# DeepLearnPhysics/dynamic-gcnn

Measured on AMD Instinct MI355X. Metric: point-clouds/sec fwd+bwd at (B,N,k,C)=(24,2048,20,3), 1/2/4/8 MI355X, higher is better.
Workload: dtype f32

## Files before the change

dynamic-gcnn_amd/csrc/bn.hip:

```cpp
#include "common.h"
#include <stdlib.h>

namespace {

constexpr int FIN_COLS = 4, FIN_LANES = 64;
__device__ __forceinline__ bool slot_sums(const double* __restrict__ acc, int F, int nslots, int& f, double& s, double& q,
                                          int colblock) {
  const int c = threadIdx.x / FIN_LANES, z = threadIdx.x % FIN_LANES;
  f = colblock * FIN_COLS + c;
  if (f >= F) return false;
  double a = 0.0, b = 0.0;
  int sl = z;
  for (; sl + 3 * FIN_LANES < nslots; sl += 4 * FIN_LANES) {
    double va[4], vb[4];
#pragma unroll
    for (int u = 0; u < 4; ++u) {
      va[u] = acc[((int64_t)(sl + u * FIN_LANES) * 2 + 0) * F + f];
      vb[u] = acc[((int64_t)(sl + u * FIN_LANES) * 2 + 1) * F + f];
    }
#pragma unroll
    for (int u = 0; u < 4; ++u) { a += va[u]; b += vb[u]; }
  }
  for (; sl < nslots; sl += FIN_LANES) {
    a += acc[((int64_t)sl * 2 + 0) * F + f];
// ... 68 lines not shown

struct Src {
  const float* Y;
  const float* V; int64_t ldv;
  const float* U; int64_t ldu;
  const int32_t* idx;
  unsigned npts;
};

#ifndef BN_NB
#define BN_NB 4
#endif
constexpr int CNT_POS = 256;
constexpr int NB = BN_NB;

template <int V, bool G>
struct Rows {
  const float* base;
  const int32_t* ip;
  int64_t ld;
  float u[V];
  __device__ __forceinline__ void init(const Src& s, int64_t r, int k, int F, int f) {
    if (G) {
      const unsigned cloud = (unsigned)r / s.npts;
      base = s.V + (int64_t)cloud * s.npts * s.ldv + f;
      ip = s.idx + r * k;
      ld = s.ldv;
      Vec<V>::ld(s.U + r * s.ldu + f, u);
    } else {
      base = s.Y + (r * k) * F + f;
      ip = nullptr;
      ld = F;
    }
  }
  __device__ __forceinline__ void load(int m, int k, float (&y)[NB][V]) const {
    if constexpr (G) {
      unsigned row[NB];
#pragma unroll
      for (int b = 0; b < NB; ++b) row[b] = __umul24((unsigned)ip[(m + b < k) ? (m + b) : (k - 1)], (unsigned)ld);
#pragma unroll
      for (int b = 0; b < NB; ++b) Vec<V>::ld(base + row[b], y[b]);
#pragma unroll
      for (int b = 0; b < NB; ++b)
#pragma unroll
        for (int v = 0; v < V; ++v) y[b][v] += u[v];
    } else {
#pragma unroll
      for (int b = 0; b < NB; ++b)
        if (m + b < k) Vec<V>::ld(base + (int64_t)(m + b) * ld, y[b]);
    }
  }
};

struct Items { int64_t base, count, first, step; };
template <bool G>
__device__ __forceinline__ Items items_of(int64_t R, int FV) {
  Items it;
  if (G) {
    const int64_t per = (R + 7) / 8;
    const int64_t rb = (int64_t)(blockIdx.x & 7) * per;
    int64_t rows = R - rb;
    rows = rows < 0 ? 0 : (rows > per ? per : rows);
    it.base = rb * FV;
    it.count = rows * FV;
    it.first = (int64_t)(blockIdx.x >> 3) * blockDim.x + threadIdx.x;
    it.step = (int64_t)(gridDim.x >> 3) * blockDim.x;
  } else {
    it.base = 0;
    it.count = R * FV;
    it.first = (int64_t)blockIdx.x * blockDim.x + threadIdx.x;
    it.step = (int64_t)gridDim.x * blockDim.x;
  }
  return it;
}

template <int V, bool G>
__global__ __launch_bounds__(256) void bn_act_kreduce_kernel(
    Src src, int64_t R, int k, int F, const float* __restrict__ mean,
    const float* __restrict__ rstd, const float* __restrict__ beta, int relu,
    float* __restrict__ max_out, int64_t ldmax, float* __restrict__ mean_out, int64_t ldmean,
    float* __restrict__ out2, int64_t ldout2, float* __restrict__ cnt_out, int fv_shift) {
  const int FV = F / V;
  const Items its = items_of<G>(R, FV);
  const float invk = 1.0f / (float)k;
  for (int64_t q = its.first; q < its.count; q += its.step) {
    int64_t r;
    int fq;
    split_item(its.base + q, FV, fv_shift, r, fq);
    const int f = fq * V;
    float mu[V], rs[V], be[V], mx[V], sm[V], cn[V], np[V];
    Vec<V>::ld(mean + f, mu); Vec<V>::ld(rstd + f, rs); Vec<V>::ld(beta + f, be);
#pragma unroll
    for (int v = 0; v < V; ++v) { mx[v] = -INFINITY; sm[v] = 0.f; cn[v] = 0.f; np[v] = 0.f; }
    Rows<V, G> rows;
    rows.init(src, r, k, F, f);
    for (int m = 0; m < k; m += NB) {
      float yv[NB][V];
      rows.load(m, k, yv);
#pragma unroll
      for (int b = 0; b < NB; ++b)
        if (m + b < k) {
#pragma unroll
          for (int v = 0; v < V; ++v) {
            float xh;
            const float z = bn_z(yv[b][v], mu[v], rs[v], be[v], relu, xh);
            const bool gt = z > mx[v];
            cn[v] = gt ? 1.f : ((z == mx[v]) ? cn[v] + 1.f : cn[v]);
            mx[v] = gt ? z : mx[v];
            sm[v] += z;
            if (G) np[v] += (z > 0.f) ? (float)CNT_POS : 0.f;
          }
        }
    }
    Vec<V>::st(max_out + r * ldmax + f, mx);
    if (out2) Vec<V>::st(out2 + r * ldout2 + f, mx);
    if (G) {
#pragma unroll
      for (int v = 0; v < V; ++v) cn[v] += np[v];
    }
    if (cnt_out) Vec<V>::st(cnt_out + r * F + f, cn);
    if (mean_out) {
#pragma unroll
      for (int v = 0; v < V; ++v) sm[v] *= invk;
      Vec<V>::st(mean_out + r * ldmean + f, sm);
    }
  }
}

template <int V>
struct KState { float mx[V]; float cnt[V]; };

template <int V, bool G>
__device__ __forceinline__ void k_pass_max(const Rows<V, G>& rows, int k, const float (&mu)[V],
                                           const float (&rs)[V], const float (&be)[V], int relu,
                                           KState<V>& st) {
#pragma unroll
  for (int v = 0; v < V; ++v) { st.mx[v] = -INFINITY; st.cnt[v] = 0.f; }
  for (int m = 0; m < k; m += NB) {
    float yv[NB][V];
    rows.load(m, k, yv);
#pragma unroll
    for (int b = 0; b < NB; ++b)
      if (m + b < k) {
#pragma unroll
        for (int v = 0; v < V; ++v) {
          float xh;
          const float z = bn_z(yv[b][v], mu[v], rs[v], be[v], relu, xh);
          if (z > st.mx[v]) { st.mx[v] = z; st.cnt[v] = 1.f; }
          else if (z == st.mx[v]) st.cnt[v] += 1.f;
        }
      }
  }
}

template <int V, bool G>
__global__ __launch_bounds__(256) void bn_bwd_reduce_kernel(
    Src src, int64_t R, int k, int F, const float* __restrict__ mean,
    const float* __restrict__ rstd, const float* __restrict__ beta, int relu,
    const float* __restrict__ dmax, int64_t lddmax, const float* __restrict__ dmean, int64_t lddmean,
    const float* __restrict__ mx_in, int64_t ldmx, const float* __restrict__ cnt_in, double* __restrict__ red,
    int fv_shift, int nslots) {
  extern __shared__ float lred[];
  for (int e = threadIdx.x; e < 2 * F; e += blockDim.x) lred[e] = 0.f;
  __syncthreads();
  const int FV = F / V;
  const Items its = items_of<G>(R, FV);
  const float invk = 1.0f / (float)k;
  int curf = -1;
  float s0[V], s1[V];
#pragma unroll
  for (int v = 0; v < V; ++v) { s0[v] = 0.f; s1[v] = 0.f; }
  for (int64_t q = its.first; q < its.count; q += its.step) {
    int64_t r;
    int fq;
    split_item(its.base + q, FV, fv_shift, r, fq);
    const int f = fq * V;
    if (f != curf) {
      if (curf >= 0) {
#pragma unroll
        for (int v = 0; v < V; ++v) { atomicAdd(&lred[curf + v], s0[v]); atomicAdd(&lred[F + curf + v], s1[v]); s0[v] = 0.f; s1[v] = 0.f; }
      }
      curf = f;
    }
    float mu[V], rs[V], be[V], dmx[V], dmn[V];
    Vec<V>::ld(mean + f, mu); Vec<V>::ld(rstd + f, rs); Vec<V>::ld(beta + f, be);
    Vec<V>::ld(dmax + r * lddmax + f, dmx);
    Rows<V, G> rows;
    rows.init(src, r, k, F, f);
    KState<V> st;
    if (dmean) {
      Vec<V>::ld(dmean + r * lddmean + f, dmn);
      if (mx_in) {
        Vec<V>::ld(mx_in + r * ldmx + f, st.mx);
        Vec<V>::ld(cnt_in + r * F + f, st.cnt);
        if (G) {
#pragma unroll
          for (int v = 0; v < V; ++v) st.cnt[v] -= (float)CNT_POS * floorf(st.cnt[v] * (1.0f / CNT_POS));
        }
      } else {
        k_pass_max<V, G>(rows, k, mu, rs, be, relu, st);
      }
    }
    for (int m = 0; m < k; m += NB) {
      float yv[NB][V];
      rows.load(m, k, yv);
#pragma unroll
      for (int b = 0; b < NB; ++b)
        if (m + b < k) {
#pragma unroll
          for (int v = 0; v < V; ++v) {
            float xh;
            const float z = bn_z(yv[b][v], mu[v], rs[v], be[v], relu, xh);
            float dz;
            if (dmean) dz = ((z == st.mx[v]) ? dmx[v] / st.cnt[v] : 0.f) + dmn[v] * invk;
            else dz = dmx[v];
            if (relu && !(z > 0.f)) dz = 0.f;
            s0[v] += dz;
            s1[v] += dz * xh;
          }
        }
    }
  }
  if (curf >= 0) {
#pragma unroll
    for (int v = 0; v < V; ++v) { atomicAdd(&lred[curf + v], s0[v]); atomicAdd(&lred[F + curf + v], s1[v]); }
  }
  __syncthreads();
  const int slot = blockIdx.x % nslots;
  for (int e = threadIdx.x; e < 2 * F; e += blockDim.x)
    atomicAdd(red + (int64_t)slot * 2 * F + e, (double)lred[e]);
}

template <int V, bool G>
__global__ __launch_bounds__(256) void bn_bwd_apply_kernel(
    Src src, int64_t R, int k, int F, const float* __restrict__ mean,
    const float* __restrict__ rstd, const float* __restrict__ beta, int relu,
    const float* __restrict__ dmax, int64_t lddmax, const float* __restrict__ dmean, int64_t lddmean,
    const float* __restrict__ mx_in, int64_t ldmx, const float* __restrict__ cnt_in,
    const double* __restrict__ red, float* dY, float* __restrict__ dYsum, int64_t lddysum, int fv_shift) {
  const bool round_dy = (relu & 2) != 0;
  relu &= 1;
  const int FV = F / V;
  const Items its = items_of<G>(R, FV);
  const float invk = 1.0f / (float)k;
  const double inv_cnt = 1.0 / ((double)R * (double)k);
  for (int64_t q = its.first; q < its.count; q += its.step) {
    int64_t r;
    int fq;
    split_item(its.base + q, FV, fv_shift, r, fq);
    const int f = fq * V;
    float mu[V], rs[V], be[V], dmx[V], dmn[V], c1[V], c2[V], acc[V];
    Vec<V>::ld(mean + f, mu); Vec<V>::ld(rstd + f, rs); Vec<V>::ld(beta + f, be);
    Vec<V>::ld(dmax + r * lddmax + f, dmx);
#pragma unroll
    for (int v = 0; v < V; ++v) {
      c1[v] = (float)(red[f + v] * inv_cnt);
      c2[v] = (float)(red[F + f + v] * inv_cnt);
      acc[v] = 0.f;
    }
    Rows<V, G> rows;
    rows.init(src, r, k, F, f);
    float* dy = dY + (r * k) * F + f;
    KState<V> st;
    if (dmean) {
      Vec<V>::ld(dmean + r * lddmean + f, dmn);
      if (mx_in) {
        Vec<V>::ld(mx_in + r * ldmx + f, st.mx);
        Vec<V>::ld(cnt_in + r * F + f, st.cnt);
        if (G) {
#pragma unroll
          for (int v = 0; v < V; ++v) st.cnt[v] -= (float)CNT_POS * floorf(st.cnt[v] * (1.0f / CNT_POS));
        }
      } else {
        k_pass_max<V, G>(rows, k, mu, rs, be, relu, st);
      }
    }
    for (int m = 0; m < k; m += NB) {
      float yv[NB][V];
      rows.load(m, k, yv);
#pragma unroll
      for (int b = 0; b < NB; ++b)
        if (m + b < k) {
          float o[V];
#pragma unroll
          for (int v = 0; v < V; ++v) {
            float xh;
            const float z = bn_z(yv[b][v], mu[v], rs[v], be[v], relu, xh);
            float dz;
            if (dmean) dz = ((z == st.mx[v]) ? dmx[v] / st.cnt[v] : 0.f) + dmn[v] * invk;
            else dz = dmx[v];
            if (relu && !(z > 0.f)) dz = 0.f;
            o[v] = rs[v] * (dz - c1[v] - xh * c2[v]);
            if (round_dy) o[v] = round_bf16_rne(o[v]);
            acc[v] += o[v];
          }
          Vec<V>::st(dy + (int64_t)(m + b) * F, o);
        }
    }
    if (dYsum) Vec<V>::st(dYsum + r * lddysum + f, acc);
  }
}


template <int CC>
__global__ __launch_bounds__(256) void edge_bwd_apply_wgrad_kernel(
    Src src, int64_t R, int k, int F, const float* __restrict__ mean, const float* __restrict__ rstd,
    const float* __restrict__ beta, const float* __restrict__ dmax, int64_t lddmax, const float* __restrict__ dmean,
    int64_t lddmean, const float* __restrict__ mx_in, int64_t ldmx, const float* __restrict__ cnt_in,
    const double* __restrict__ red, const float* __restrict__ x, int64_t ldx, int C, float* __restrict__ partial, int fv_shift) {
  constexpr int V = 4;
  extern __shared__ float sh[];
  const int FV = F / V;
  const Items its = items_of<true>(R, FV);
  const float invk = 1.0f / (float)k;
  const double inv_cnt = 1.0 / ((double)R * (double)k);
  float wc[CC][V], wd[CC][V];
#pragma unroll
  for (int c = 0; c < CC; ++c)
#pragma unroll
    for (int v = 0; v < V; ++v) { wc[c][v] = 0.f; wd[c][v] = 0.f; }
  const int fq_fixed = (int)((its.base + its.first) & (FV - 1));
  const int f = fq_fixed * V;
  float mu[V], rs[V], be[V], c1[V], c2[V];
  Vec<V>::ld(mean + f, mu); Vec<V>::ld(rstd + f, rs); Vec<V>::ld(beta + f, be);
#pragma unroll
  for (int v = 0; v < V; ++v) {
    c1[v] = (float)(red[f + v] * inv_cnt);
    c2[v] = (float)(red[F + f + v] * inv_cnt);
  }
  for (int64_t q = its.first; q < its.count; q += its.step) {
    const int64_t r = (its.base + q) >> fv_shift;
    float dmx[V], dmn[V];
    Vec<V>::ld(dmax + r * lddmax + f, dmx);
    Vec<V>::ld(dmean + r * lddmean + f, dmn);
    Rows<V, true> rows;
    rows.init(src, r, k, F, f);
    KState<V> st;
    Vec<V>::ld(mx_in + r * ldmx + f, st.mx);
    Vec<V>::ld(cnt_in + r * F + f, st.cnt);
#pragma unroll
    for (int v = 0; v < V; ++v) st.cnt[v] -= (float)CNT_POS * floorf(st.cnt[v] * (1.0f / CNT_POS));
    float xi[CC];
#pragma unroll
    for (int c = 0; c < CC; ++c) xi[c] = (c < C) ? x[r * ldx + c] : 0.f;
    const int64_t cloud0 = (int64_t)((unsigned)r / src.npts) * src.npts;
    float acc[V] = {0.f, 0.f, 0.f, 0.f};
    for (int m = 0; m < k; m += NB) {
      float yv[NB][V];
      rows.load(m, k, yv);
#pragma unroll
      for (int b = 0; b < NB; ++b)
        if (m + b < k) {
          const float* xj = x + (cloud0 + rows.ip[m + b]) * ldx;
          float dx[CC];
#pragma unroll
          for (int c = 0; c < CC; ++c) dx[c] = (c < C) ? xj[c] - xi[c] : 0.f;
#pragma unroll
          for (int v = 0; v < V; ++v) {
            float xh;
            const float z = bn_z(yv[b][v], mu[v], rs[v], be[v], 1, xh);
            float dz = ((z == st.mx[v]) ? dmx[v] / st.cnt[v] : 0.f) + dmn[v] * invk;
            if (!(z > 0.f)) dz = 0.f;
            const float o = rs[v] * (dz - c1[v] - xh * c2[v]);
            acc[v] += o;
#pragma unroll
            for (int c = 0; c < CC; ++c) wd[c][v] = fmaf(dx[c], o, wd[c][v]);
          }
        }
    }
#pragma unroll
    for (int c = 0; c < CC; ++c)
#pragma unroll
      for (int v = 0; v < V; ++v) wc[c][v] = fmaf(xi[c], acc[v], wc[c][v]);
  }
  const int lanes = 256 / FV;
  const int rl = threadIdx.x / FV;
#pragma unroll
  for (int c = 0; c < CC; ++c)
#pragma unroll
    for (int v = 0; v < V; ++v) {
      sh[(rl * 2 * CC + c) * F + f + v] = wc[c][v];
      sh[(rl * 2 * CC + CC + c) * F + f + v] = wd[c][v];
    }
  __syncthreads();
  float* out = partial + (int64_t)blockIdx.x * 2 * C * F;
  for (int e = threadIdx.x; e < 2 * CC * F; e += 256) {
    const int cr = e / F, ff = e % F;
    const int c = cr < CC ? cr : cr - CC;
    if (c >= C) continue;
    float s = 0.f;
    for (int l = 0; l < lanes; ++l) s += sh[(l * 2 * CC + cr) * F + ff];
    out[(int64_t)(cr < CC ? c : C + c) * F + ff] = s;
  }
}

struct K1Map {
  int f; int64_t r0, rstep; bool on;
};
__device__ __forceinline__ K1Map k1_map(int F, int FVB, int RP) {
  K1Map m;
  const int t = threadIdx.x;
  const int fq = blockIdx.y * 256 + (t % FVB);
  m.f = fq * 4;
  m.on = (t < RP * FVB) && (m.f < F);
  m.r0 = (int64_t)blockIdx.x * RP + t / FVB;
  m.rstep = (int64_t)gridDim.x * RP;
  return m;
}

constexpr int K1_PARK_FLOATS = 2048;
__device__ __forceinline__ void k1_block_sums(float* lpark, const K1Map& m, int F, int FVB, int RP, const float (&s0)[4],
                                              const float (&s1)[4], double* __restrict__ red, int nslots) {
  const int t = threadIdx.x;
  const int W = 4 * FVB;
  if (t < RP * FVB) {
    const int rp = t / FVB, cb = (t % FVB) * 4;
#pragma unroll
    for (int v = 0; v < 4; ++v) {
      lpark[(rp * 2 + 0) * W + cb + v] = m.on ? s0[v] : 0.f;
      lpark[(rp * 2 + 1) * W + cb + v] = m.on ? s1[v] : 0.f;
    }
  }
  __syncthreads();
  const int fbase = blockIdx.y * 1024;
  const int slot = blockIdx.x % nslots;
  for (int e = t; e < 2 * W; e += blockDim.x) {
    const int which = e / W, cb = e % W;
    if (fbase + cb < F) {
      float a = 0.f;
      for (int rp = 0; rp < RP; ++rp) a += lpark[(rp * 2 + which) * W + cb];
      atomicAdd(red + ((int64_t)slot * 2 + which) * F + fbase + cb, (double)a);
    }
  }
}

__global__ __launch_bounds__(256) void bn1_act_kernel(const float* __restrict__ T, int64_t R, int F, int FVB, int RP,
                                                      const float* __restrict__ mean, const float* __restrict__ rstd,
                                                      const float* __restrict__ beta, int relu,
                                                      float* __restrict__ out, int64_t ldo, float* __restrict__ out2,
                                                      int64_t ldo2, float* __restrict__ cnt_out,
                                                      const uint64_t* __restrict__ drop_seed, float drop_keep) {
  const K1Map m = k1_map(F, FVB, RP);
  if (!m.on) return;
  const uint64_t dseed = drop_seed ? *drop_seed : 0ull;
  const uint32_t dthr = dropout_threshold(drop_keep);
  const float dscale = drop_seed ? 1.0f / drop_keep : 1.0f;
  float mu[4], rs[4], be[4];
  Vec<4>::ld(mean + m.f, mu); Vec<4>::ld(rstd + m.f, rs); Vec<4>::ld(beta + m.f, be);
  const float one[4] = {1.f, 1.f, 1.f, 1.f};
  for (int64_t r = m.r0; r < R; r += 4 * m.rstep) {
    float y[4][4];
#pragma unroll
    for (int b = 0; b < 4; ++b) {
      const int64_t rr = r + b * m.rstep;
      if (rr < R) Vec<4>::ld(T + rr * F + m.f, y[b]);
    }
#pragma unroll
    for (int b = 0; b < 4; ++b) {
      const int64_t rr = r + b * m.rstep;
      if (rr < R) {
        float z[4];
#pragma unroll
        for (int v = 0; v < 4; ++v) { float xh; z[v] = bn_z(y[b][v], mu[v], rs[v], be[v], relu, xh); }
        if (drop_seed) {
#pragma unroll
          for (int v = 0; v < 4; ++v) z[v] = dropout_keeps(dseed, (uint64_t)(rr * F + m.f + v), dthr) ? z[v] * dscale : 0.f;
        }
        Vec<4>::st(out + rr * ldo + m.f, z);
        if (out2) Vec<4>::st(out2 + rr * ldo2 + m.f, z);
        if (cnt_out) Vec<4>::st(cnt_out + rr * F + m.f, one);
      }
    }
  }
}

template <bool APPLY>
__global__ __launch_bounds__(256) void bn1_bwd_kernel(const float* T, int64_t R, int F, int FVB, int RP,
                                                      const float* __restrict__ mean, const float* __restrict__ rstd,
                                                      const float* __restrict__ beta, int relu,
                                                      const float* __restrict__ dout, int64_t lddo,
                                                      const float* __restrict__ dout2, int64_t lddo2,
                                                      double* __restrict__ red, float* dT, float* __restrict__ dsum,
                                                      int64_t lddsum, const uint64_t* __restrict__ drop_seed, float drop_keep,
                                                      int nslots) {
  extern __shared__ float lred[];
  const uint64_t dseed = drop_seed ? *drop_seed : 0ull;
  const uint32_t dthr = dropout_threshold(drop_keep);
  const float dscale = drop_seed ? 1.0f / drop_keep : 1.0f;
  const K1Map m = k1_map(F, FVB, RP);
  float mu[4] = {0, 0, 0, 0}, rs[4] = {0, 0, 0, 0}, be[4] = {0, 0, 0, 0}, c1[4] = {0, 0, 0, 0}, c2[4] = {0, 0, 0, 0};
  float s0[4] = {0, 0, 0, 0}, s1[4] = {0, 0, 0, 0};
  if (m.on) {
    Vec<4>::ld(mean + m.f, mu); Vec<4>::ld(rstd + m.f, rs); Vec<4>::ld(beta + m.f, be);
    if (APPLY) {
      const double inv_cnt = 1.0 / (double)R;
#pragma unroll
      for (int v = 0; v < 4; ++v) {
        c1[v] = (float)(red[m.f + v] * inv_cnt);
        c2[v] = (float)(red[F + m.f + v] * inv_cnt);
      }
    }
    for (int64_t r = m.r0; r < R; r += 4 * m.rstep) {
      float y[4][4], d[4][4];
#pragma unroll
      for (int b = 0; b < 4; ++b) {
        const int64_t rr = r + b * m.rstep;
        if (rr < R) {
          Vec<4>::ld(T + rr * F + m.f, y[b]); Vec<4>::ld(dout + rr * lddo + m.f, d[b]);
          if (dout2) {
            float e[4];
            Vec<4>::ld(dout2 + rr * lddo2 + m.f, e);
#pragma unroll
            for (int v = 0; v < 4; ++v) d[b][v] += e[v];
          }
        }
      }
#pragma unroll
      for (int b = 0; b < 4; ++b) {
        const int64_t rr = r + b * m.rstep;
        if (rr < R) {
          float o[4];
#pragma unroll
          for (int v = 0; v < 4; ++v) {
            float xh;
            const float z = bn_z(y[b][v], mu[v], rs[v], be[v], relu, xh);
            float dz = d[b][v];
            if (drop_seed) dz = dropout_keeps(dseed, (uint64_t)(rr * F + m.f + v), dthr) ? dz * dscale : 0.f;
            if (relu && !(z > 0.f)) dz = 0.f;
            if (APPLY) o[v] = rs[v] * (dz - c1[v] - xh * c2[v]);
            else { s0[v] += dz; s1[v] += dz * xh; }
          }
          if (APPLY) {
            Vec<4>::st(dT + rr * F + m.f, o);
            if (dsum) Vec<4>::st(dsum + rr * lddsum + m.f, o);
          }
        }
      }
    }
  }
  if (!APPLY) k1_block_sums(lred, m, F, FVB, RP, s0, s1, red, nslots);
}


template <int N>
__global__ __launch_bounds__(256) void bn1_act_class_kernel(const float* __restrict__ T, int64_t R,
                                                            const float* __restrict__ mean, const float* __restrict__ rstd,
                                                            const float* __restrict__ beta, int relu,
                                                            float* __restrict__ out, int64_t ldo,
                                                            const uint64_t* __restrict__ drop_seed, float drop_keep,
                                                            const float* __restrict__ W, int64_t ldw,
                                                            float* __restrict__ C, int64_t ldc, double* __restrict__ stats,
                                                            int nslots, float* __restrict__ scal) {
  constexpr int F = 256;
  __shared__ float bs[F * N + 8 * N];
  float* red = bs + F * N;
  for (int e = threadIdx.x; e < F * N; e += 256) bs[e] = W[(int64_t)(e / N) * ldw + (e % N)];
  if (scal && blockIdx.x == 0 && threadIdx.x < 2) scal[threadIdx.x] = 0.f;
  __syncthreads();
  const int lane = threadIdx.x & 63, wv = threadIdx.x >> 6;
  const int f = lane * 4;
  const int64_t rstep = (int64_t)gridDim.x * 4;
  const uint64_t dseed = *drop_seed;
  const uint32_t dthr = dropout_threshold(drop_keep);
  const float dscale = 1.0f / drop_keep;
  float mu[4], rs[4], be[4];
  Vec<4>::ld(mean + f, mu); Vec<4>::ld(rstd + f, rs); Vec<4>::ld(beta + f, be);
  float cs[N], cq[N];
#pragma unroll
  for (int n = 0; n < N; ++n) { cs[n] = 0.f; cq[n] = 0.f; }
  for (int64_t r = (int64_t)blockIdx.x * 4 + wv; r < R; r += 4 * rstep) {
    float y[4][4];
#pragma unroll
    for (int b = 0; b < 4; ++b) {
      const int64_t rr = r + b * rstep;
      if (rr < R) Vec<4>::ld(T + rr * F + f, y[b]);
    }
#pragma unroll
    for (int b = 0; b < 4; ++b) {
      const int64_t rr = r + b * rstep;
      if (rr < R) {
        float z[4];
#pragma unroll
        for (int v = 0; v < 4; ++v) { float xh; z[v] = bn_z(y[b][v], mu[v], rs[v], be[v], relu, xh); }
#pragma unroll
        for (int v = 0; v < 4; ++v) z[v] = dropout_keeps(dseed, (uint64_t)(rr * F + f + v), dthr) ? z[v] * dscale : 0.f;
        Vec<4>::st(out + rr * ldo + f, z);
        float acc[N];
#pragma unroll
        for (int n = 0; n < N; ++n) acc[n] = 0.f;
        skinny_nn_chunk<N>(acc, make_float4(z[0], z[1], z[2], z[3]), bs + f * N);
        skinny_nn_tree<N>(acc);
        if (lane == 0) {
#pragma unroll
          for (int n = 0; n < N; ++n) {
            const float v = acc[n];
            C[rr * ldc + n] = v;
            cs[n] += v;
            cq[n] += v * v;
          }
        }
      }
    }
  }
  if (lane == 0) {
#pragma unroll
    for (int n = 0; n < N; ++n) { red[wv * 2 * N + n] = cs[n]; red[wv * 2 * N + N + n] = cq[n]; }
  }
  __syncthreads();
  if (threadIdx.x < 2 * N) {
    const int which = threadIdx.x / N, n = threadIdx.x % N;
    const float a = ((red[threadIdx.x] + red[2 * N + threadIdx.x]) + red[4 * N + threadIdx.x]) + red[6 * N + threadIdx.x];
    atomicAdd(stats + ((int64_t)(blockIdx.x % nslots) * 2 + which) * N + n, (double)a);
  }
}

__global__ __launch_bounds__(256) void bn_softmax_xent_kernel(const float* __restrict__ Y, const double* __restrict__ stats,
                                                              int nslots, double count, float eps,
                                                              const float* __restrict__ beta, int relu, int64_t rows, int ncls,
                                                              float* __restrict__ mean, float* __restrict__ rstd, float* fin,
                                                              const int32_t* __restrict__ labels,
                                                              const float* __restrict__ weight, float* __restrict__ softmax,
                                                              float* __restrict__ dlogits, float* __restrict__ scal) {
  __shared__ float sl[256], sc[256];
  __shared__ float smu[FIN_COLS], srs[FIN_COLS];
  {
    int f;
    double s, q;
    if (slot_sums(stats, ncls, nslots, f, s, q, 0)) {
      const double mu = s / count;
      double var = q / count - mu * mu;
      if (var < 0.0) var = 0.0;
      smu[f] = (float)mu;
      srs[f] = (float)(1.0 / sqrt(var + (double)eps));
      if (blockIdx.x == 0) { mean[f] = smu[f]; rstd[f] = srs[f]; }
    }
  }
  __syncthreads();
  float loss = 0.f, corr = 0.f;
  const float inv_rows = 1.0f / (float)rows;
  for (int64_t r = (int64_t)blockIdx.x * blockDim.x + threadIdx.x; r < rows; r += (int64_t)gridDim.x * blockDim.x) {
    float* z = fin + r * ncls;
    for (int c = 0; c < ncls; ++c) { float xh; z[c] = bn_z(Y[r * ncls + c], smu[c], srs[c], beta[c], relu, xh); }
    const int lab = labels ? labels[r] : -1;
    const float w = weight ? weight[r] : 1.f;
    softmax_xent_row(z, ncls, lab, w, inv_rows, softmax ? softmax + r * ncls : nullptr,
                     dlogits ? dlogits + r * ncls : nullptr, loss, corr);
  }
  sl[threadIdx.x] = loss;
  sc[threadIdx.x] = corr;
  __syncthreads();
  for (int s = 128; s > 0; s >>= 1) {
    if ((int)threadIdx.x < s) { sl[threadIdx.x] += sl[threadIdx.x + s]; sc[threadIdx.x] += sc[threadIdx.x + s]; }
    __syncthreads();
  }
  if (threadIdx.x == 0 && scal) {
    atomicAdd(scal + 0, sl[0] * inv_rows);
    atomicAdd(scal + 1, sc[0] * inv_rows);
  }
}

template <bool APPLY, int NC>
__global__ __launch_bounds__(256) void bn1_bwd_class_kernel(const float* T, int64_t R, const float* __restrict__ mean,
                                                            const float* __restrict__ rstd, const float* __restrict__ beta,
                                                            int relu, const uint64_t* __restrict__ drop_seed, float drop_keep,
                                                            float* Tf, const float* __restrict__ mean_f,
                                                            const float* __restrict__ rstd_f, const float* __restrict__ beta_f,
                                                            int relu_f, const float* __restrict__ dfin,
                                                            const double* __restrict__ red_f, int nslots_f,
                                                            float* __restrict__ dbeta_f, float dbeta_f_beta,
                                                            const float* __restrict__ W, int64_t ldw,
                                                            double* __restrict__ red, float* dT, int nslots) {
  constexpr int F = 256, FVB = 64, RP = 4;
  extern __shared__ float lred[];
  __shared__ float sc1[FIN_COLS], sc2[FIN_COLS];
  const uint64_t dseed = *drop_seed;
  const uint32_t dthr = dropout_threshold(drop_keep);
  const float dscale = 1.0f / drop_keep;
  const K1Map m = k1_map(F, FVB, RP);
  float muf[NC], rsf[NC], bef[NC], c1f[NC], c2f[NC];
  if (!APPLY) {
    int f;
// ... 191 lines not shown
  return dg::check_launch(what);
}

template <bool G>
int launch_bwd_reduce(const char* what, Src src, int64_t R, int k, int F, const float* mean, const float* rstd,
                      const float* beta, int relu, const float* dmax, int64_t lddmax, const float* dmean,
                      int64_t lddmean, const float* mx_in, int64_t ldmx, const float* cnt_in, double* red,
                      hipStream_t st) {
  DG_REQUIRE(mean && rstd && beta && dmax && red, DGCNN_EINVAL, "%s: null pointer", what);
  DG_REQUIRE(F <= 8192, DGCNN_EINVAL, "%s: F > 8192", what);
  DG_REQUIRE(!mx_in || cnt_in, DGCNN_EINVAL, "%s: mx_in needs cnt_in", what);
  DG_REQUIRE(relu == 0 || relu == 1, DGCNN_EINVAL, "%s: relu must be 0 or 1 (got %d; the bf16 flag belongs to the apply pass)", what, relu);
  const bool vec = (F % 4 == 0) && (lddmax % 4 == 0) && (G || a16(src.Y)) && a16(dmax) && a16(mean) && a16(rstd) &&
                   a16(beta) && (!dmean || ((lddmean % 4 == 0) && a16(dmean))) &&
                   (!mx_in || ((ldmx % 4 == 0) && a16(mx_in) && a16(cnt_in)));
  const size_t sh = (size_t)2 * F * sizeof(float);
  if (G) {
    DG_REQUIRE(vec, DGCNN_EINVAL, "%s: operands must be 16-byte aligned with leading dimensions %% 4 == 0", what);
    dg::launch((bn_bwd_reduce_kernel<4, true>), dim3(grid8(grid_reduce(R * (F / 4)))), dim3(256), sh, st, src, R, k,
                       F, mean, rstd, beta, relu, dmax, lddmax, dmean, lddmean, mx_in, ldmx, cnt_in, red, shift_of(F / 4), dg::stat_slots());
  } else if (vec && k == 1 && !mx_in) {
    const int mb = 256;
    const K1Grid g = k1_grid(R, F, mb);
    const size_t sh1 = sizeof(float) * K1_PARK_FLOATS;
    dg::launch((bn1_bwd_kernel<false>), g.grid, dim3(256), sh1, st, src.Y, R, F, g.FVB, g.RP, mean, rstd, beta, relu,
                       dmax, lddmax, dmean, lddmean, red, (float*)nullptr, (float*)nullptr, (int64_t)0, (const uint64_t*)nullptr, 1.0f,
                       dg::stat_slots());
  } else if (vec) {
    dg::launch((bn_bwd_reduce_kernel<4, false>), dim3(grid_reduce(R * (F / 4))), dim3(256), sh, st, src, R, k, F,
                       mean, rstd, beta, relu, dmax, lddmax, dmean, lddmean, mx_in, ldmx, cnt_in, red, shift_of(F / 4), dg::stat_slots());
  } else {
    dg::launch((bn_bwd_reduce_kernel<1, false>), dim3(grid_reduce(R * F)), dim3(256), sh, st, src, R, k, F, mean,
                       rstd, beta, relu, dmax, lddmax, dmean, lddmean, mx_in, ldmx, cnt_in, red, shift_of(F), dg::stat_slots());
  }
  return dg::check_launch(what);
}

template <bool G>
int launch_bwd_apply(const char* what, Src src, int64_t R, int k, int F, const float* mean, const float* rstd,
                     const float* beta, int relu, const float* dmax, int64_t lddmax, const float* dmean,
                     int64_t lddmean, const float* mx_in, int64_t ldmx, const float* cnt_in, double* red, float* dY,
                     float* dYsum, int64_t lddysum, float* dbeta, float dbeta_beta, hipStream_t st) {
  DG_REQUIRE(mean && rstd && beta && dmax && red && dY, DGCNN_EINVAL, "%s: null pointer", what);
  DG_REQUIRE(!dYsum || lddysum >= F, DGCNN_EINVAL, "%s: lddysum < F", what);
  DG_REQUIRE(relu >= 0 && relu <= 3, DGCNN_EINVAL, "%s: relu must be 0 .. 3 (bit 0 = ReLU, bit 1 = bf16 dY; got %d)", what, relu);
  dg::launch(bn_bwd_finalize_kernel, dim3((unsigned)dg::cdiv(F, FIN_COLS)), dim3(FIN_COLS * FIN_LANES), 0, st, red, F, dg::stat_slots(), dbeta,
                     dbeta_beta);
  const bool vec = (F % 4 == 0) && (lddmax % 4 == 0) && (G || a16(src.Y)) && a16(dY) && a16(dmax) && a16(mean) &&
                   a16(rstd) && a16(beta) && (!dmean || ((lddmean % 4 == 0) && a16(dmean))) &&
                   (!dYsum || (a16(dYsum) && lddysum % 4 == 0)) &&
                   (!mx_in || ((ldmx % 4 == 0) && a16(mx_in) && a16(cnt_in)));
  if (G) {
    DG_REQUIRE(vec, DGCNN_EINVAL, "%s: operands must be 16-byte aligned with leading dimensions %% 4 == 0", what);
    dg::launch((bn_bwd_apply_kernel<4, true>), dim3(grid8(grid_for(R * (F / 4)))), dim3(256), 0, st, src, R, k, F,
                       mean, rstd, beta, relu, dmax, lddmax, dmean, lddmean, mx_in, ldmx, cnt_in, red, dY, dYsum, lddysum,
                       shift_of(F / 4));
  } else if (vec && k == 1 && !mx_in && !(relu & 2)) {
    const K1Grid g = k1_grid(R, F, 4096);
    dg::launch((bn1_bwd_kernel<true>), g.grid, dim3(256), 0, st, src.Y, R, F, g.FVB, g.RP, mean, rstd, beta, relu,
                       dmax, lddmax, dmean, lddmean, red, dY, dYsum, lddysum, (const uint64_t*)nullptr, 1.0f, dg::stat_slots());
  } else if (vec) {
    dg::launch((bn_bwd_apply_kernel<4, false>), dim3(grid_for(R * (F / 4))), dim3(256), 0, st, src, R, k, F, mean,
                       rstd, beta, relu, dmax, lddmax, dmean, lddmean, mx_in, ldmx, cnt_in, red, dY, dYsum, lddysum,
                       shift_of(F / 4));
  } else {
    dg::launch((bn_bwd_apply_kernel<1, false>), dim3(grid_for(R * F)), dim3(256), 0, st, src, R, k, F, mean, rstd,
                       beta, relu, dmax, lddmax, dmean, lddmean, mx_in, ldmx, cnt_in, red, dY, dYsum, lddysum, shift_of(F));
  }
  return dg::check_launch(what);
}

}

extern "C" int dgcnn_bn_finalize_f32(const double* stats, int F, double count, float eps,
                                     float* mean, float* rstd, void* stream) {
  DG_REQUIRE(stats && mean && rstd && F > 0 && count > 0, DGCNN_EINVAL, "dgcnn_bn_finalize_f32: bad args");
  dg::launch(bn_finalize_kernel, dim3((unsigned)dg::cdiv(F, FIN_COLS)), dim3(FIN_COLS * FIN_LANES), 0, (hipStream_t)stream,
                     stats, F, dg::stat_slots(), count, eps, mean, rstd);
  return dg::check_launch("dgcnn_bn_finalize_f32");
}

extern "C" int dgcnn_bn_act_kreduce_f32(const float* Y, int64_t R, int k, int F,
                                        const float* mean, const float* rstd, const float* beta, int relu,
                                        float* max_out, int64_t ldmax, float* mean_out, int64_t ldmean,
                                        float* out2, int64_t ldout2, float* cnt_out, void* stream) {
  DG_REQUIRE(Y, DGCNN_EINVAL, "dgcnn_bn_act_kreduce_f32: null pointer");
  DG_REQUIRE(R > 0 && k > 0 && F > 0, DGCNN_EINVAL, "dgcnn_bn_act_kreduce_f32: bad shape");
  return launch_act_kreduce<false>("dgcnn_bn_act_kreduce_f32", dense_src(Y), R, k, F, mean, rstd, beta, relu, max_out,
                                   ldmax, mean_out, ldmean, out2, ldout2, cnt_out, (hipStream_t)stream);
}

extern "C" int dgcnn_bn_bwd_reduce_f32(const float* Y, int64_t R, int k, int F,
                                       const float* mean, const float* rstd, const float* beta, int relu,
                                       const float* dmax, int64_t lddmax, const float* dmean, int64_t lddmean,
                                       const float* mx_in, int64_t ldmx, const float* cnt_in,
                                       double* red, void* stream) {
  DG_REQUIRE(Y, DGCNN_EINVAL, "dgcnn_bn_bwd_reduce_f32: null pointer");
  DG_REQUIRE(R > 0 && k > 0 && F > 0, DGCNN_EINVAL, "dgcnn_bn_bwd_reduce_f32: bad shape");
  return launch_bwd_reduce<false>("dgcnn_bn_bwd_reduce_f32", dense_src(Y), R, k, F, mean, rstd, beta, relu, dmax, lddmax,
                                  dmean, lddmean, mx_in, ldmx, cnt_in, red, (hipStream_t)stream);
}

extern "C" int dgcnn_bn_bwd_apply_f32(const float* Y, int64_t R, int k, int F,
                                      const float* mean, const float* rstd, const float* beta, int relu,
                                      const float* dmax, int64_t lddmax, const float* dmean, int64_t lddmean,
                                      const float* mx_in, int64_t ldmx, const float* cnt_in,
                                      double* red, float* dY, float* dYsum, int64_t lddysum, float* dbeta,
                                      float dbeta_beta, void* stream) {
  DG_REQUIRE(Y, DGCNN_EINVAL, "dgcnn_bn_bwd_apply_f32: null pointer");
  DG_REQUIRE(R > 0 && k > 0 && F > 0, DGCNN_EINVAL, "dgcnn_bn_bwd_apply_f32: bad shape");
  return launch_bwd_apply<false>("dgcnn_bn_bwd_apply_f32", dense_src(Y), R, k, F, mean, rstd, beta, relu, dmax, lddmax,
                                 dmean, lddmean, mx_in, ldmx, cnt_in, red, dY, dYsum, lddysum, dbeta, dbeta_beta,
                                 (hipStream_t)stream);
}

extern "C" int dgcnn_edge_bn_act_kreduce_f32(const float* V, int64_t ldv, const float* U, int64_t ldu,
                                             const int32_t* idx, int B, int N, int k, int F,
                                             const float* mean, const float* rstd, const float* beta, int relu,
                                             float* max_out, int64_t ldmax, float* mean_out, int64_t ldmean,
                                             float* cnt_out, void* stream) {
  int rc = check_edge("dgcnn_edge_bn_act_kreduce_f32", V, ldv, U, ldu, idx, B, N, k, F);
  if (rc) return rc;
  return launch_act_kreduce<true>("dgcnn_edge_bn_act_kreduce_f32", edge_src(V, ldv, U, ldu, idx, N), (int64_t)B * N, k, F,
                                  mean, rstd, beta, relu, max_out, ldmax, mean_out, ldmean, nullptr, 0, cnt_out,
                                  (hipStream_t)stream);
}

extern "C" int dgcnn_edge_bn_bwd_reduce_f32(const float* V, int64_t ldv, const float* U, int64_t ldu,
                                            const int32_t* idx, int B, int N, int k, int F,
                                            const float* mean, const float* rstd, const float* beta, int relu,
                                            const float* dmax, int64_t lddmax, const float* dmean, int64_t lddmean,
                                            const float* mx_in, int64_t ldmx, const float* cnt_in,
                                            double* red, void* stream) {
  int rc = check_edge("dgcnn_edge_bn_bwd_reduce_f32", V, ldv, U, ldu, idx, B, N, k, F);
  if (rc) return rc;
  return launch_bwd_reduce<true>("dgcnn_edge_bn_bwd_reduce_f32", edge_src(V, ldv, U, ldu, idx, N), (int64_t)B * N, k, F,
                                 mean, rstd, beta, relu, dmax, lddmax, dmean, lddmean, mx_in, ldmx, cnt_in, red,
                                 (hipStream_t)stream);
}

extern "C" int dgcnn_edge_bn_bwd_reduce_points_f32(const float* mx, int64_t ldmx, const float* mn, int64_t ldmn,
                                                   const float* cntpos, const float* dmax, int64_t lddmax,
                                                   const float* dmean, int64_t lddmean, const float* beta,
                                                   int64_t R, int k, int F, double* red, void* stream) {
  DG_REQUIRE(mx && mn && cntpos && dmax && dmean && beta && red, DGCNN_EINVAL, "dgcnn_edge_bn_bwd_reduce_points_f32: null pointer");
  DG_REQUIRE(R > 0 && k > 0 && k < CNT_POS && F > 0 && F % 4 == 0, DGCNN_EINVAL,
             "dgcnn_edge_bn_bwd_reduce_points_f32: bad shape (F %% 4 == 0, k < %d)", CNT_POS);
  DG_REQUIRE(a16(mx) && a16(mn) && a16(cntpos) && a16(dmax) && a16(dmean) && a16(beta) && ldmx % 4 == 0 && ldmn % 4 == 0 &&
                 lddmax % 4 == 0 && lddmean % 4 == 0, DGCNN_EINVAL,
             "dgcnn_edge_bn_bwd_reduce_points_f32: operands must be 16-byte aligned with leading dimensions %% 4 == 0");
  const K1Grid g = k1_grid(R, F, 256);
  const size_t sh = sizeof(float) * K1_PARK_FLOATS;
  dg::launch(edge_bwd_reduce_points_kernel, g.grid, dim3(256), sh, (hipStream_t)stream, mx, ldmx, mn, ldmn, cntpos,
                     dmax, lddmax, dmean, lddmean, beta, R, k, F, g.FVB, g.RP, red, dg::stat_slots());
  return dg::check_launch("dgcnn_edge_bn_bwd_reduce_points_f32");
}

extern "C" int dgcnn_edge_bn_bwd_apply_f32(const float* V, int64_t ldv, const float* U, int64_t ldu,
                                           const int32_t* idx, int B, int N, int k, int F,
                                           const float* mean, const float* rstd, const float* beta, int relu,
                                           const float* dmax, int64_t lddmax, const float* dmean, int64_t lddmean,
                                           const float* mx_in, int64_t ldmx, const float* cnt_in,
                                           double* red, float* dY, float* dYsum, int64_t lddysum, float* dbeta,
                                           float dbeta_beta, void* stream) {
  int rc = check_edge("dgcnn_edge_bn_bwd_apply_f32", V, ldv, U, ldu, idx, B, N, k, F);
  if (rc) return rc;
  return launch_bwd_apply<true>("dgcnn_edge_bn_bwd_apply_f32", edge_src(V, ldv, U, ldu, idx, N), (int64_t)B * N, k, F, mean,
                                rstd, beta, relu, dmax, lddmax, dmean, lddmean, mx_in, ldmx, cnt_in, red, dY, dYsum,
                                lddysum, dbeta, dbeta_beta, (hipStream_t)stream);
}

static int check_bn1_drop(const char* what, const float* T, int64_t R, int F, const float* mean, const float* rstd,
                          const float* beta, int relu, float keep, const uint64_t* seed_dev) {
  DG_REQUIRE(relu == 0 || relu == 1, DGCNN_EINVAL, "%s: relu must be 0 or 1 (got %d)", what, relu);
  DG_REQUIRE(T && mean && rstd && beta && seed_dev && R > 0 && F > 0 && keep > 0.f && keep <= 1.f, DGCNN_EINVAL, "%s: bad args", what);
  DG_REQUIRE(F % 4 == 0 && a16(T) && a16(mean) && a16(rstd) && a16(beta), DGCNN_EUNSUP, "%s: F %% 4 == 0 and 16-byte aligned operands required", what);
  return DGCNN_OK;
}

extern "C" int dgcnn_bn1_act_dropout_f32(const float* T, int64_t R, int F, const float* mean, const float* rstd,
                                         const float* beta, int relu, float keep, const uint64_t* seed_dev, float* out,
                                         int64_t ldo, void* stream) {
  int rc = check_bn1_drop("dgcnn_bn1_act_dropout_f32", T, R, F, mean, rstd, beta, relu, keep, seed_dev);
  if (rc) return rc;
  DG_REQUIRE(out && ldo % 4 == 0 && a16(out), DGCNN_EINVAL, "dgcnn_bn1_act_dropout_f32: out must be 16-byte aligned, ld %% 4 == 0");
  const K1Grid g = k1_grid(R, F, 4096);
  dg::launch(bn1_act_kernel, g.grid, dim3(256), 0, (hipStream_t)stream, T, R, F, g.FVB, g.RP, mean, rstd, beta, relu, out,
                     ldo, (float*)nullptr, (int64_t)0, (float*)nullptr, seed_dev, keep);
  return dg::check_launch("dgcnn_bn1_act_dropout_f32");
}

extern "C" int dgcnn_bn1_bwd_dropout_f32(const float* T, int64_t R, int F, const float* mean, const float* rstd,
                                         const float* beta, int relu, float keep, const uint64_t* seed_dev,
                                         const float* dout, int64_t lddo, double* red, float* dT, float* dbeta,
                                         float dbeta_beta, void* stream) {
  int rc = check_bn1_drop("dgcnn_bn1_bwd_dropout_f32", T, R, F, mean, rstd, beta, relu, keep, seed_dev);
  if (rc) return rc;
  DG_REQUIRE(dout && red && dT && lddo % 4 == 0 && a16(dout) && a16(dT) && F <= 8192, DGCNN_EINVAL, "dgcnn_bn1_bwd_dropout_f32: bad args");
  hipStream_t st = (hipStream_t)stream;
  const K1Grid gr = k1_grid(R, F, 256);
  const size_t sh1 = sizeof(float) * K1_PARK_FLOATS;
  dg::launch((bn1_bwd_kernel<false>), gr.grid, dim3(256), sh1, st, T, R, F, gr.FVB, gr.RP, mean, rstd, beta, relu, dout, lddo,
                     (const float*)nullptr, (int64_t)0, red, (float*)nullptr, (float*)nullptr, (int64_t)0, seed_dev, keep, dg::stat_slots());
  dg::launch(bn_bwd_finalize_kernel, dim3((unsigned)dg::cdiv(F, FIN_COLS)), dim3(FIN_COLS * FIN_LANES), 0, st, red, F, dg::stat_slots(), dbeta, dbeta_beta);
  const K1Grid ga = k1_grid(R, F, 4096);
  dg::launch((bn1_bwd_kernel<true>), ga.grid, dim3(256), 0, st, T, R, F, ga.FVB, ga.RP, mean, rstd, beta, relu, dout, lddo,
                     (const float*)nullptr, (int64_t)0, red, dT, (float*)nullptr, (int64_t)0, seed_dev, keep, dg::stat_slots());
  return dg::check_launch("dgcnn_bn1_bwd_dropout_f32");
}

static int check_class_tail(const char* what, int F, int ncls, const float* W, int64_t ldw) {
  DG_REQUIRE(F == 256, DGCNN_EUNSUP, "%s: the last FC layer must be 256 wide (got %d): one wave per row", what, F);
  DG_REQUIRE(ncls >= 1 && ncls <= 4, DGCNN_EUNSUP, "%s: 1 .. 4 classes (got %d)", what, ncls);
  DG_REQUIRE(W && ldw >= ncls, DGCNN_EINVAL, "%s: bad class weight", what);
  return DGCNN_OK;
}

extern "C" int dgcnn_bn1_act_class_f32(const float* T, int64_t R, int F, const float* mean, const float* rstd,
                                       const float* beta, int relu, float keep, const uint64_t* seed_dev, float* out,
                                       int64_t ldo, const float* W, int64_t ldw, int ncls, float* logits, int64_t ldc,
                                       double* stats, float* scal, void* stream) {
  int rc = check_bn1_drop("dgcnn_bn1_act_class_f32", T, R, F, mean, rstd, beta, relu, keep, seed_dev);
  if (rc) return rc;
  rc = check_class_tail("dgcnn_bn1_act_class_f32", F, ncls, W, ldw);
  if (rc) return rc;
  DG_REQUIRE(out && ldo % 4 == 0 && ldo >= F && a16(out), DGCNN_EINVAL, "dgcnn_bn1_act_class_f32: out must be 16-byte aligned, ld %% 4 == 0");
  DG_REQUIRE(logits && ldc >= ncls && stats && R < (1ll << 31), DGCNN_EINVAL, "dgcnn_bn1_act_class_f32: bad logits / stats");
  const unsigned g = (unsigned)dg::cap_writers(dg::cdiv(R, 4) < 2048 ? dg::cdiv(R, 4) : 2048);
  hipStream_t st = (hipStream_t)stream;
#define DG_ACT_CLASS(NN) dg::launch((bn1_act_class_kernel<NN>), dim3(g), dim3(256), 0, st, T, R, mean, rstd, beta, relu, out, ldo, \
                                    seed_dev, keep, W, ldw, logits, ldc, stats, dg::stat_slots(), scal)
  if (ncls == 1) DG_ACT_CLASS(1); else if (ncls == 2) DG_ACT_CLASS(2); else if (ncls == 3) DG_ACT_CLASS(3); else DG_ACT_CLASS(4);
#undef DG_ACT_CLASS
  return dg::check_launch("dgcnn_bn1_act_class_f32");
}

extern "C" int dgcnn_bn_softmax_xent_f32(const float* Y, const double* stats, double count, float eps, const float* beta,
                                         int relu, int64_t rows, int ncls, float* mean, float* rstd, float* fin,
                                         const int32_t* labels, const float* weight, float* softmax, float* dlogits,
                                         float* scal, void* stream) {
  DG_REQUIRE(Y && stats && beta && mean && rstd && fin && rows > 0 && count > 0, DGCNN_EINVAL, "dgcnn_bn_softmax_xent_f32: bad args");
  DG_REQUIRE(ncls >= 1 && ncls <= FIN_COLS, DGCNN_EUNSUP, "dgcnn_bn_softmax_xent_f32: 1 .. %d classes (got %d)", FIN_COLS, ncls);
  DG_REQUIRE(relu == 0 || relu == 1, DGCNN_EINVAL, "dgcnn_bn_softmax_xent_f32: relu must be 0 or 1 (got %d)", relu);
  DG_REQUIRE(!dlogits || labels, DGCNN_EINVAL, "dgcnn_bn_softmax_xent_f32: dlogits needs labels");
  int64_t g = dg::cdiv(rows, 256);
  if (g > 1024) g = 1024;
  dg::launch(bn_softmax_xent_kernel, dim3((unsigned)g), dim3(256), 0, (hipStream_t)stream, Y, stats, dg::stat_slots(), count, eps,
             beta, relu, rows, ncls, mean, rstd, fin, labels, weight, softmax, dlogits, scal);
  return dg::check_launch("dgcnn_bn_softmax_xent_f32");
}

extern "C" int dgcnn_bn1_bwd_class_f32(const float* T, int64_t R, int F, const float* mean, const float* rstd,
                                       const float* beta, int relu, float keep, const uint64_t* seed_dev, float* Tf, int ncls,
                                       const float* mean_f, const float* rstd_f, const float* beta_f, int relu_f,
                                       const float* dfin, double* red_f, float* dbeta_f, float dbeta_f_beta, const float* W,
                                       int64_t ldw, double* red, float* dT, float* dbeta, float dbeta_beta, int phases, void* stream) {
  DG_REQUIRE(phases >= 1 && phases <= 3, DGCNN_EINVAL, "dgcnn_bn1_bwd_class_f32: phases must be 1 (sums), 2 (finalize + dT) or 3 (got %d)", phases);
  int rc = check_bn1_drop("dgcnn_bn1_bwd_class_f32", T, R, F, mean, rstd, beta, relu, keep, seed_dev);
  if (rc) return rc;
  rc = check_class_tail("dgcnn_bn1_bwd_class_f32", F, ncls, W, ldw);
  if (rc) return rc;
  DG_REQUIRE(Tf && mean_f && rstd_f && beta_f && dfin && red_f && red && dT && a16(dT) && (relu_f == 0 || relu_f == 1), DGCNN_EINVAL,
             "dgcnn_bn1_bwd_class_f32: bad args");
  hipStream_t st = (hipStream_t)stream;
  const K1Grid gr = k1_grid(R, F, 256);
  const K1Grid ga = k1_grid(R, F, 4096);
  const size_t sh1 = sizeof(float) * K1_PARK_FLOATS;
  const int ns = dg::stat_slots();
#define DG_BWD_CLASS(NC)                                                                                                         \
  do {                                                                                                                           \
    if (phases & 1)                                                                                                              \
      dg::launch((bn1_bwd_class_kernel<false, NC>), gr.grid, dim3(256), sh1, st, T, R, mean, rstd, beta, relu, seed_dev, keep,    \
                 Tf, mean_f, rstd_f, beta_f, relu_f, dfin, red_f, ns, dbeta_f, dbeta_f_beta, W, ldw, red, (float*)nullptr, ns);   \
    if (!(phases & 2)) break;                                                                                                    \
    dg::launch(bn_bwd_finalize_kernel, dim3((unsigned)dg::cdiv(F, FIN_COLS)), dim3(FIN_COLS * FIN_LANES), 0, st, red, F, ns,     \
               dbeta, dbeta_beta);                                                                                               \
    dg::launch((bn1_bwd_class_kernel<true, NC>), ga.grid, dim3(256), 0, st, T, R, mean, rstd, beta, relu, seed_dev, keep, Tf,     \
               mean_f, rstd_f, beta_f, relu_f, dfin, red_f, ns, (float*)nullptr, 0.f, W, ldw, red, dT, ns);                       \
  } while (0)
  if (ncls == 1) DG_BWD_CLASS(1); else if (ncls == 2) DG_BWD_CLASS(2); else if (ncls == 3) DG_BWD_CLASS(3); else DG_BWD_CLASS(4);
#undef DG_BWD_CLASS
  return dg::check_launch("dgcnn_bn1_bwd_class_f32");
}

namespace dg {
void launch_reduce_partials(const float* part, int splits, int M, int N, float* C, int64_t ldc, float beta, hipStream_t st);
void launch_bn_bwd_finalize(double* red, int F, float* dbeta, float dbeta_beta, hipStream_t st) {
  dg::launch(bn_bwd_finalize_kernel, dim3((unsigned)cdiv(F, FIN_COLS)), dim3(FIN_COLS * FIN_LANES), 0, st, red, F, stat_slots(), dbeta, dbeta_beta);
}
}

extern "C" int dgcnn_edge_bn_bwd_apply_wgrad_f32(const float* V, int64_t ldv, const float* U, int64_t ldu,
                                                 const int32_t* idx, int B, int N, int k, int F,
                                                 const float* mean, const float* rstd, const float* beta,
                                                 const float* dmax, int64_t lddmax, const float* dmean, int64_t lddmean,
                                                 const float* mx_in, int64_t ldmx, const float* cnt_in, double* red,
                                                 const float* x, int64_t ldx, int C, float* dW0, float* dbeta,
                                                 float dbeta_beta, void* ws, size_t ws_bytes, void* stream) {
  int rc = check_edge("dgcnn_edge_bn_bwd_apply_wgrad_f32", V, ldv, U, ldu, idx, B, N, k, F);
  if (rc) return rc;
  DG_REQUIRE(mean && rstd && beta && dmax && dmean && mx_in && cnt_in && red && x && dW0 && ws, DGCNN_EINVAL,
             "dgcnn_edge_bn_bwd_apply_wgrad_f32: null pointer");
  DG_REQUIRE(C >= 1 && C <= 4, DGCNN_EUNSUP, "dgcnn_edge_bn_bwd_apply_wgrad_f32: C must be <= 4 (got %d)", C);
  const int FV = F / 4;
  DG_REQUIRE(shift_of(FV) >= 0 && FV <= 256 && lddmax % 4 == 0 && lddmean % 4 == 0 && ldmx % 4 == 0 && a16(dmax) && a16(dmean) &&
                 a16(mx_in) && a16(cnt_in) && a16(mean) && a16(rstd) && a16(beta), DGCNN_EUNSUP,
             "dgcnn_edge_bn_bwd_apply_wgrad_f32: F / 4 must be a power of two <= 256, operands 16-byte aligned");
  hipStream_t st = (hipStream_t)stream;
  const int64_t R = (int64_t)B * N;
  dg::launch(bn_bwd_finalize_kernel, dim3((unsigned)dg::cdiv(F, FIN_COLS)), dim3(FIN_COLS * FIN_LANES), 0, st, red, F, dg::stat_slots(), dbeta, dbeta_beta);
  const unsigned grid = grid8(grid_reduce(R * FV));
  const size_t need = (size_t)grid * 2 * C * F * sizeof(float);
  DG_REQUIRE(ws_bytes >= need, DGCNN_ENOSPC, "dgcnn_edge_bn_bwd_apply_wgrad_f32: workspace too small (%zu < %zu)", ws_bytes, need);
  const size_t shb = (size_t)(256 / FV) * 2 * 4 * F * sizeof(float);
  dg::launch((edge_bwd_apply_wgrad_kernel<4>), dim3(grid), dim3(256), shb, st, edge_src(V, ldv, U, ldu, idx, N), R, k, F,
                     mean, rstd, beta, dmax, lddmax, dmean, lddmean, mx_in, ldmx, cnt_in, red, x, ldx, C,
                     reinterpret_cast<float*>(ws), shift_of(FV));
  rc = dg::check_launch("dgcnn_edge_bn_bwd_apply_wgrad_f32");
  if (rc) return rc;
  dg::launch_reduce_partials(reinterpret_cast<const float*>(ws), (int)grid, 2 * C, F, dW0, (int64_t)F, 1.0f, st);
  return dg::check_launch("dgcnn_edge_bn_bwd_apply_wgrad_f32(reduce)");
}
```

Baseline: 5456.

## Specialize edge BN-backward wgrad kernel on channel count and streamline neighbor loop

The fused edge BN-backward plus weight-gradient kernel is now templated on the actual input channel count C. This removes padded work and registers for unused channels, and the launch picks one of four instantiations. The inner neighbor loop processes two edges at a time with direct vector loads and 24-bit index multiplies. Per-row quotients (dmax/cnt, dmean/k) are hoisted out of that loop, and the kernel requests four blocks per CU to push occupancy. A new host check limits ldx and N*ldx so the 32-bit offsets stay valid; the kernel now relies on Rows internals (base, u, ld) instead of its load helper.

```diff
diff --git a/dynamic-gcnn_amd/csrc/bn.hip b/dynamic-gcnn_amd/csrc/bn.hip
--- a/dynamic-gcnn_amd/csrc/bn.hip
+++ b/dynamic-gcnn_amd/csrc/bn.hip
@@ -394,21 +394,23 @@
 }
 
 
-template <int CC>
-__global__ __launch_bounds__(256) void edge_bwd_apply_wgrad_kernel(
+template <int C>
+__global__ __launch_bounds__(256, 4) void edge_bwd_apply_wgrad_kernel(
     Src src, int64_t R, int k, int F, const float* __restrict__ mean, const float* __restrict__ rstd,
     const float* __restrict__ beta, const float* __restrict__ dmax, int64_t lddmax, const float* __restrict__ dmean,
     int64_t lddmean, const float* __restrict__ mx_in, int64_t ldmx, const float* __restrict__ cnt_in,
-    const double* __restrict__ red, const float* __restrict__ x, int64_t ldx, int C, float* __restrict__ partial, int fv_shift) {
+    const double* __restrict__ red, const float* __restrict__ x, int64_t ldx, float* __restrict__ partial, int fv_shift) {
   constexpr int V = 4;
+  constexpr int NBW = 2;
+  constexpr int CC = 4;
   extern __shared__ float sh[];
   const int FV = F / V;
   const Items its = items_of<true>(R, FV);
   const float invk = 1.0f / (float)k;
   const double inv_cnt = 1.0 / ((double)R * (double)k);
-  float wc[CC][V], wd[CC][V];
-#pragma unroll
-  for (int c = 0; c < CC; ++c)
+  float wc[C][V], wd[C][V];
+#pragma unroll
+  for (int c = 0; c < C; ++c)
 #pragma unroll
     for (int v = 0; v < V; ++v) { wc[c][v] = 0.f; wd[c][v] = 0.f; }
   const int fq_fixed = (int)((its.base + its.first) & (FV - 1));
@@ -422,53 +424,70 @@
   }
   for (int64_t q = its.first; q < its.count; q += its.step) {
     const int64_t r = (its.base + q) >> fv_shift;
-    float dmx[V], dmn[V];
-    Vec<V>::ld(dmax + r * lddmax + f, dmx);
-    Vec<V>::ld(dmean + r * lddmean + f, dmn);
+    const int fi = (int)((its.base + q) & (FV - 1)) * V;
     Rows<V, true> rows;
-    rows.init(src, r, k, F, f);
-    KState<V> st;
-    Vec<V>::ld(mx_in + r * ldmx + f, st.mx);
-    Vec<V>::ld(cnt_in + r * F + f, st.cnt);
-#pragma unroll
-    for (int v = 0; v < V; ++v) st.cnt[v] -= (float)CNT_POS * floorf(st.cnt[v] * (1.0f / CNT_POS));
-    float xi[CC];
-#pragma unroll
-    for (int c = 0; c < CC; ++c) xi[c] = (c < C) ? x[r * ldx + c] : 0.f;
-    const int64_t cloud0 = (int64_t)((unsigned)r / src.npts) * src.npts;
+    rows.init(src, r, k, F, fi);
+    float mx[V], dq[V], dn[V];
+    {
+      float dmx[V], dmn[V], cnt[V];
+      Vec<V>::ld(dmax + r * lddmax + fi, dmx);
+      Vec<V>::ld(dmean + r * lddmean + fi, dmn);
+      Vec<V>::ld(mx_in + r * ldmx + fi, mx);
+      Vec<V>::ld(cnt_in + r * F + fi, cnt);
+#pragma unroll
+      for (int v = 0; v < V; ++v) {
+        cnt[v] -= (float)CNT_POS * floorf(cnt[v] * (1.0f / CNT_POS));
+        dq[v] = dmx[v] / cnt[v];
+        dn[v] = dmn[v] * invk;
+      }
+    }
+    float xi[C];
+#pragma unroll
+    for (int c = 0; c < C; ++c) xi[c] = x[r * ldx + c];
+    const float* xb = x + (int64_t)((unsigned)r / src.npts) * src.npts * ldx;
     float acc[V] = {0.f, 0.f, 0.f, 0.f};
-    for (int m = 0; m < k; m += NB) {
-      float yv[NB][V];
-      rows.load(m, k, yv);
-#pragma unroll
-      for (int b = 0; b < NB; ++b)
-        if (m + b < k) {
-          const float* xj = x + (cloud0 + rows.ip[m + b]) * ldx;
-          float dx[CC];
-#pragma unroll
-          for (int c = 0; c < CC; ++c) dx[c] = (c < C) ? xj[c] - xi[c] : 0.f;
-#pragma unroll
-          for (int v = 0; v < V; ++v) {
-            float xh;
-            const float z = bn_z(yv[b][v], mu[v], rs[v], be[v], 1, xh);
-            float dz = ((z == st.mx[v]) ? dmx[v] / st.cnt[v] : 0.f) + dmn[v] * invk;
-            if (!(z > 0.f)) dz = 0.f;
-            const float o = rs[v] * (dz - c1[v] - xh * c2[v]);
-            acc[v] += o;
-#pragma unroll
-            for (int c = 0; c < CC; ++c) wd[c][v] = fmaf(dx[c], o, wd[c][v]);
-          }
+    for (int m = 0; m < k; m += NBW) {
+      unsigned j[NBW];
+#pragma unroll
+      for (int b = 0; b < NBW; ++b) j[b] = (unsigned)rows.ip[(m + b < k) ? (m + b) : (k - 1)];
+      float yv[NBW][V];
+#pragma unroll
+      for (int b = 0; b < NBW; ++b) Vec<V>::ld(rows.base + __umul24(j[b], (unsigned)rows.ld), yv[b]);
+      auto edge = [&](int b) {
+        const float* xj = xb + __umul24(j[b], (unsigned)ldx);
+        float dx[C];
+#pragma unroll
+        for (int c = 0; c < C; ++c) dx[c] = xj[c] - xi[c];
+#pragma unroll
+        for (int v = 0; v < V; ++v) {
+          float xh;
+          const float z = bn_z(yv[b][v] + rows.u[v], mu[v], rs[v], be[v], 1, xh);
+          float dz = ((z == mx[v]) ? dq[v] : 0.f) + dn[v];
+          if (!(z > 0.f)) dz = 0.f;
+          const float o = rs[v] * (dz - c1[v] - xh * c2[v]);
+          acc[v] += o;
+#pragma unroll
+          for (int c = 0; c < C; ++c) wd[c][v] = fmaf(dx[c], o, wd[c][v]);
         }
-    }
-#pragma unroll
-    for (int c = 0; c < CC; ++c)
+      };
+      if (m + NBW <= k) {
+#pragma unroll
+        for (int b = 0; b < NBW; ++b) edge(b);
+      } else {
+#pragma unroll
+        for (int b = 0; b < NBW; ++b)
+          if (m + b < k) edge(b);
+      }
+    }
+#pragma unroll
+    for (int c = 0; c < C; ++c)
 #pragma unroll
       for (int v = 0; v < V; ++v) wc[c][v] = fmaf(xi[c], acc[v], wc[c][v]);
   }
   const int lanes = 256 / FV;
   const int rl = threadIdx.x / FV;
 #pragma unroll
-  for (int c = 0; c < CC; ++c)
+  for (int c = 0; c < C; ++c)
 #pragma unroll
     for (int v = 0; v < V; ++v) {
       sh[(rl * 2 * CC + c) * F + f + v] = wc[c][v];
@@ -1266,6 +1285,8 @@
   DG_REQUIRE(mean && rstd && beta && dmax && dmean && mx_in && cnt_in && red && x && dW0 && ws, DGCNN_EINVAL,
              "dgcnn_edge_bn_bwd_apply_wgrad_f32: null pointer");
   DG_REQUIRE(C >= 1 && C <= 4, DGCNN_EUNSUP, "dgcnn_edge_bn_bwd_apply_wgrad_f32: C must be <= 4 (got %d)", C);
+  DG_REQUIRE(ldx >= C && ldx < (1 << 24) && (int64_t)N * ldx < (1ll << 32), DGCNN_EUNSUP,
+             "dgcnn_edge_bn_bwd_apply_wgrad_f32: ldx >= C and N * ldx < 2^32 elements (32-bit row offsets inside a cloud)");
   const int FV = F / 4;
   DG_REQUIRE(shift_of(FV) >= 0 && FV <= 256 && lddmax % 4 == 0 && lddmean % 4 == 0 && ldmx % 4 == 0 && a16(dmax) && a16(dmean) &&
                  a16(mx_in) && a16(cnt_in) && a16(mean) && a16(rstd) && a16(beta), DGCNN_EUNSUP,
@@ -1277,9 +1298,11 @@
   const size_t need = (size_t)grid * 2 * C * F * sizeof(float);
   DG_REQUIRE(ws_bytes >= need, DGCNN_ENOSPC, "dgcnn_edge_bn_bwd_apply_wgrad_f32: workspace too small (%zu < %zu)", ws_bytes, need);
   const size_t shb = (size_t)(256 / FV) * 2 * 4 * F * sizeof(float);
-  dg::launch((edge_bwd_apply_wgrad_kernel<4>), dim3(grid), dim3(256), shb, st, edge_src(V, ldv, U, ldu, idx, N), R, k, F,
-                     mean, rstd, beta, dmax, lddmax, dmean, lddmean, mx_in, ldmx, cnt_in, red, x, ldx, C,
-                     reinterpret_cast<float*>(ws), shift_of(FV));
+#define DG_APPLY_WGRAD(NC) dg::launch((edge_bwd_apply_wgrad_kernel<NC>), dim3(grid), dim3(256), shb, st, edge_src(V, ldv, U, ldu, idx, N), \
+                                     R, k, F, mean, rstd, beta, dmax, lddmax, dmean, lddmean, mx_in, ldmx, cnt_in, red, x, ldx,         \
+                                     reinterpret_cast<float*>(ws), shift_of(FV))
+  if (C == 1) DG_APPLY_WGRAD(1); else if (C == 2) DG_APPLY_WGRAD(2); else if (C == 3) DG_APPLY_WGRAD(3); else DG_APPLY_WGRAD(4);
+#undef DG_APPLY_WGRAD
   rc = dg::check_launch("dgcnn_edge_bn_bwd_apply_wgrad_f32");
   if (rc) return rc;
   dg::launch_reduce_partials(reinterpret_cast<const float*>(ws), (int)grid, 2 * C, F, dW0, (int64_t)F, 1.0f, st);
```

After: 5499 (median of 6 runs). About the same (+0.8%).
